# robert80203/HuPR-A-Benchmark-for-Human-Pose-Estimation-Using-Millimeter-Wave-Radar

Hardware: AMD Instinct MI355X
Metric: radar frames/sec (FFT->heatmap fwd+bwd) (higher is better)
Workload: dtype bf16

## Files before the change

hupr-a-benchmark-for-human-pose-estimation-using-millimeter-wave-radar_amd/csrc/conv_halo.h:

```cpp
#pragma once
#include "gemm_common.h"

namespace hupr {

typedef __bf16 bf16x8 __attribute__((ext_vector_type(8)));
typedef unsigned u32x4 __attribute__((ext_vector_type(4)));
typedef float f32x4n __attribute__((ext_vector_type(4)));

typedef __bf16 bf16x4 __attribute__((ext_vector_type(4)));

struct HaloArgs {
    const void* x;
    const __bf16* wp;
    const float* bias;
    const void* res;
    void* y;
    int Bn, D, H, W, Ci, in_ld, Co, out_ld, res_ld;
    int kd;
    int TD, log2TW;
    int nd, nh, nw;
    int n_co_tiles;
    int ablate;
    unsigned long long* trace;
    double* stats;
    float* part;
    int units_per_slice;
    int no_res_prefetch;
};

__device__ __forceinline__ void halo_store_partial(const HaloArgs& p, const f32x16& acc, long m, int chb, int slice) {
    const long M = (long)p.Bn * p.D * p.H * p.W;
    float* dst = p.part + ((long)slice * M + m) * p.Co;
#pragma unroll
    for (int g = 0; g < 4; ++g) {
        const int ch = chb + 8 * g;
        if (ch < p.Co) *reinterpret_cast<f32x4n*>(dst + ch) = (f32x4n){acc[4 * g], acc[4 * g + 1], acc[4 * g + 2], acc[4 * g + 3]};
    }
}

enum HaloRoute {
    kRouteCi32 = 1,
    kRouteCo32 = 2,
    kRoute1x16x16 = 3,
    kRouteStats4x8x8One = 4,
    kRouteStats4x8x8Two = 5,
    kRouteStats2x8x16 = 6,
    kRoute4x8x8 = 7,
    kRoute2x8x16 = 8,
    kRoute128 = 256,
};

int conv_halo256_route(HaloArgs& a, int Bn, bool abf);
void launch_conv_halo256(const HaloArgs& a, int route, hipStream_t s);
bool conv_halo256_supported(const HaloArgs& a, int Bn, bool abf);
bool conv_halo256_stats_ok(const HaloArgs& a, int Bn);
void set_halo_tiles(int mask);
constexpr int kHalo256Grid = 256;

template <bool ABF>
__device__ __forceinline__ void halo_store_voxel(const HaloArgs& p, const f32x16& acc, long m, int chb) {
    if constexpr (ABF) {
        if ((p.Co & 7) == 0 && (p.out_ld & 7) == 0) {
            const int lh = (chb >> 2) & 1, cb = chb - 4 * lh;
            unsigned pk[4][2];
#pragma unroll
            for (int g = 0; g < 4; ++g) {
                f32x4n v = {acc[4 * g], acc[4 * g + 1], acc[4 * g + 2], acc[4 * g + 3]};
                const int ch = chb + 8 * g;
                if (p.bias && ch < p.Co) v += (f32x4n){p.bias[ch], p.bias[ch + 1], p.bias[ch + 2], p.bias[ch + 3]};
                if (p.res && ch < p.Co) {
                    const bf16x4 rv = *reinterpret_cast<const bf16x4*>(static_cast<const __bf16*>(p.res) + m * p.res_ld + ch);
                    v += (f32x4n){(float)rv[0], (float)rv[1], (float)rv[2], (float)rv[3]};
                }
                typedef __bf16 bf16x2 __attribute__((ext_vector_type(2)));
                const bf16x2 lo = {(__bf16)v[0], (__bf16)v[1]}, hi = {(__bf16)v[2], (__bf16)v[3]};
                pk[g][0] = __builtin_bit_cast(unsigned, lo);
                pk[g][1] = __builtin_bit_cast(unsigned, hi);
            }
#pragma unroll
            for (int gp = 0; gp < 4; gp += 2) {
                const auto r0 = __builtin_amdgcn_permlane32_swap(pk[gp][0], pk[gp + 1][0], false, false);
                const auto r1 = __builtin_amdgcn_permlane32_swap(pk[gp][1], pk[gp + 1][1], false, false);
                const int ch = cb + 8 * (gp + lh);
                if (ch < p.Co)
                    *reinterpret_cast<u32x4*>(static_cast<__bf16*>(p.y) + m * p.out_ld + ch) = (u32x4){r0[0], r1[0], r0[1], r1[1]};
            }
            return;
        }
    }
// ... 41 lines not shown
```

hupr-a-benchmark-for-human-pose-estimation-using-millimeter-wave-radar_amd/csrc/conv_halo256m_bf16.hip:

```cpp
#include "conv_halo.h"

namespace hupr {

typedef float f32x4c __attribute__((ext_vector_type(4)));

template <int TD, int TH, int TW, int KD, int NCOT = 0, int NWN = 2, int KC = 64>
__global__ __launch_bounds__(512) void hupr_k_conv_halo256m_bf16(HaloArgs p) {
    constexpr int LDK = KC, BN = 32 * NWN, TS = KC == 64 ? 3 : 9, C8 = KC / 8, L2C8 = KC == 64 ? 3 : 2;
    static_assert(KC == 64 || (KC == 32 && KD == 3 && NWN == 2 && NCOT == 0), "32-channel rows: 3 x 3 x 3 taps, 64 output channels per tile");
    constexpr int HD = TD + KD - 1, HH = TH + 2, HW = TW + 2;
    static_assert(TD * TH * TW == 64 * (8 / NWN) && TH % 8 == 0 && TW % 8 == 0 && (KD == 1 || KD == 3) && (NWN == 2 || NCOT == 0),
                  "256 (512) voxels per tile, 8 x 8 per wave");
    constexpr int NVOX = HD * HH * HW;
    constexpr int T = 9 * KD, NSTAGE = KC == 64 ? 3 * KD : KD, NTAP = KC == 64 ? 6 : 9;
    constexpr bool FULLD = NWN == 1;
    constexpr int NVOXL = FULLD ? TD * HH * HW : NVOX, VOX0 = FULLD ? HH * HW : 0;
    constexpr int NH = (NVOXL * C8 + 511) / 512;
    constexpr int Y0 = NH < NTAP - 1 ? NH : NTAP - 1, Y1 = NH - (NTAP - 1) < 0 ? 0 : (NH - (NTAP - 1) > NTAP ? NTAP : NH - (NTAP - 1)),
                  Y2 = NH - (2 * NTAP - 1) < 0 ? 0 : (NH - (2 * NTAP - 1) > NTAP ? NTAP : NH - (2 * NTAP - 1));
    static_assert(NH <= NTAP * NSTAGE - 1 && NH <= 3 * NTAP - 1, "halo items must all be issued in front of the item's last barrier (and within three stages)");
    __shared__ __attribute__((aligned(16))) __bf16 Hs[(KC == 32 ? 2 : 1) * NVOX * LDK];
    __shared__ __attribute__((aligned(16))) __bf16 Bs[2][TS][BN * LDK];
    constexpr bool STATS = NCOT > 0 && KD == 3;
    constexpr bool SINGLE = STATS && TD == 2;
    f32x4c ssum[STATS ? NCOT : 1][2], ssq[STATS ? NCOT : 1][2];
    if constexpr (!SINGLE) {
#pragma unroll
        for (int ct = 0; ct < (STATS ? NCOT : 1); ++ct)
#pragma unroll
            for (int cg = 0; cg < 2; ++cg) { ssum[ct][cg] = (f32x4c){0.f, 0.f, 0.f, 0.f}; ssq[ct][cg] = (f32x4c){0.f, 0.f, 0.f, 0.f}; }
    }

    const int tid = threadIdx.x, lane = tid & 63, wave = tid >> 6;
    if (wave >= 4) __builtin_amdgcn_s_setprio(1);
    const int wm = NWN == 2 ? wave >> 1 : wave, wn = NWN == 2 ? wave & 1 : 0;
    constexpr int NBX = TW / 8, NBY = TH / 8;
    const int xw0 = 8 * (wm % NBX), yw0 = 8 * ((wm / NBX) % NBY), dzw = wm / (NBX * NBY);
    const int idx = lane & 15, kq = lane >> 4, yy = idx >> 3, wx = idx & 7;
    const int n_tiles = p.Bn * p.nd * p.nh * p.nw * p.n_co_tiles;

    const int wrow_ = NWN == 2 ? 8 * wave + (lane >> 3) : ((8 * wave + (lane >> 3)) & 31);
    const int wsrc_lane = (wrow_ * T * p.Ci + (((lane & 7) ^ (wrow_ >> 1)) & 7) * 8) * 2 +
                          (NWN == 2 ? 0 : (wave >> 2) * (3 * p.Ci * 2));
    constexpr int NDMA = NWN == 2 ? TS : 2, DMA_TAPS = NWN == 2 ? 1 : 2;
    const int wrow32_ = 16 * (wave & 3) + (lane >> 2);
    const int wsrc32_lane = (wrow32_ * T * p.Ci + (((lane & 3) ^ (((wrow32_ >> 3) & 1) << 1)) & 3) * 8) * 2;
    const u32x4 wrs = {(unsigned)(unsigned long)p.wp, (unsigned)((unsigned long)p.wp >> 32) & 0xffffu,
                       (unsigned)((long)p.Co * T * p.Ci * 2), 0x00020000u};
    const unsigned bs_lds = (unsigned)(unsigned long)(__attribute__((address_space(3))) void*)&Bs[0][0][0];
    const unsigned wdst_wave = __builtin_amdgcn_readfirstlane(bs_lds + wave * 1024);
#define HUPR_W_DMA(COT_, CH_, S_, PAR_)                                                                             \
    if constexpr (KC == 32) {                                                                                       \
        _Pragma("unroll") for (int j = 0; j < 5; ++j) {                                                             \
            if (j < 4 || wave < 4) {                                                                                \
                const int t9_ = 2 * j + (wave >> 2);                                  \
                const int wb32_ = (((COT_) * BN * T + (S_) * 9 + (t9_ % 3) * 3 + t9_ / 3) * p.Ci + (CH_) * KC) * 2 + wsrc32_lane; \
                unsigned keep_;                                                                                     \
                asm volatile("s_mov_b32 %0, m0\n\ts_mov_b32 m0, %1\n\ts_nop 0\n\tbuffer_load_dwordx4 %2, %3, 0 offen lds\n\t" \
                             "s_mov_b32 m0, %0"                                                                     \
                             : "=&s"(keep_)                                                                         \
                             : "s"(wdst_wave + (PAR_) * TS * (BN * LDK * 2) + j * 8192), "v"(wb32_), "s"(wrs)       \
                             : "memory");                                                                           \
            }                                                                                                       \
        }                                                                                                           \
    } else {                                                                                                        \
        const int wbase_ = (((COT_) * BN * T + ((S_) / 3) * 9 + ((S_) % 3)) * p.Ci + (CH_) * KC) * 2 + wsrc_lane;   \
        _Pragma("unroll") for (int j = 0; j < NDMA; ++j) {                                                          \
            if (NWN == 2 || j == 0 || wave < 4) {                                                                   \
                unsigned keep_;                                                                                     \
                asm volatile("s_mov_b32 %0, m0\n\ts_mov_b32 m0, %1\n\ts_nop 0\n\tbuffer_load_dwordx4 %2, %3, 0 offen lds\n\t" \
                             "s_mov_b32 m0, %0"                                                                     \
                             : "=&s"(keep_)                                                                         \
                             : "s"(NWN == 2 ? wdst_wave + ((PAR_) * TS + j) * (BN * LDK * 2)                        \
                                            : wdst_wave + (PAR_) * TS * (BN * LDK * 2) + j * 8192),                 \
                               "v"(NWN == 2 ? wbase_ + j * (3 * p.Ci * 2) : wbase_ + j * DMA_TAPS * (3 * p.Ci * 2)), "s"(wrs) \
                             : "memory");                                                                           \
            }                                                                                                       \
        }                                                                                                           \
    }

    u32x4 vb[NH];
    const __amdgpu_buffer_rsrc_t xrs = __builtin_amdgcn_make_buffer_rsrc(
        const_cast<void*>(p.x), 0, (int)((long)p.Bn * p.D * p.H * p.W * p.in_ld * 2), 0x00020000);
#define HUPR_HALO_ISSUE_ITEM(u, COND_, B_, D0_, H0_, W0_, C0_)                                                     \
    {                                                                                                               \
        const int it = tid + (u) * 512;                                                                             \
        const int vox = it >> L2C8, c8 = it & (C8 - 1);                                                             \
        const int hx = vox % HW;                                                                                    \
        const int t_ = vox / HW;                                                                                    \
        const int hy = t_ % HH, hz = t_ / HH;                                                                       \
        const int d = (D0_) + hz - (FULLD ? 0 : KD / 2), h = (H0_) + hy - 1, w = (W0_) + hx - 1;                    \
        const bool ok = (COND_) && it < NVOXL * C8 && (unsigned)d < (unsigned)p.D && (unsigned)h < (unsigned)p.H && \
                        (unsigned)w < (unsigned)p.W;                                                                \
        const int off = (((((B_) * p.D + d) * p.H + h) * p.W + w) * p.in_ld + (C0_) + c8 * 8) * 2;                  \
        const auto ld_ = __builtin_amdgcn_raw_buffer_load_b128(xrs, ok ? off : 0x7ffffff0, 0, 0);                  \
        vb[u] = (u32x4){ld_[0], ld_[1], ld_[2], ld_[3]};                                                            \
    }
#define HUPR_HALO_COMMIT()                                                                                          \
    _Pragma("unroll") for (int u = 0; u < NH; ++u) {                                                                \
        const int it = tid + u * 512;                                                                               \
        if (it < NVOXL * C8) {                                                                                      \
            const int vox = it >> L2C8, c8 = it & (C8 - 1);                                                         \
            const int hx = vox % HW;                                                                                \
            const int key_ = KC == 64 ? (((hx >> 1) & 3) << 1) : ((((vox / HW) % HH) & 1) << 1);                    \
            *reinterpret_cast<u32x4*>(&Hs[(vox + VOX0) * LDK + ((c8 ^ key_) << 3)]) = vb[u];                        \
        }                                                                                                           \
    }

    struct Pos { int cot, twi, thi, tdi, b, ch; };
    const int n_chunks = p.Ci / KC;
    const int per_wg = (n_tiles + gridDim.x - 1) / gridDim.x;
    const int wg_rank = (int)((blockIdx.x & 7) * (gridDim.x >> 3) + (blockIdx.x >> 3));
    const int t_begin = wg_rank * per_wg, t_end = min(n_tiles, t_begin + per_wg);
    if (STATS && p.stats) {
        if (t_begin >= t_end) {
            for (int c = tid; c < 2 * p.Co; c += 512) p.stats[(long)blockIdx.x * 2 * p.Co + c] = 0.0;
        }
    }
    if (t_begin >= t_end) return;
    Pos cur;
    {
        cur.cot = t_begin % p.n_co_tiles;
        int st = t_begin / p.n_co_tiles;
        cur.twi = st % p.nw; st /= p.nw;
        cur.thi = st % p.nh; st /= p.nh;
        cur.tdi = st % p.nd;
        cur.b = st / p.nd;
        cur.ch = 0;
    }
    const int n_items = (t_end - t_begin) * n_chunks;
    const int cot0 = cur.cot;

    int woff[2][2];
#pragma unroll
    for (int cg = 0; cg < 2; ++cg)
#pragma unroll
        for (int kk = 0; kk < 2; ++kk) {
            const int n = 32 * wn + 16 * cg + idx;
            woff[cg][kk] = KC == 64 ? n * LDK + (((4 * kk + kq) ^ ((n >> 1) & 7)) << 3) : n * LDK + ((kq ^ (((n >> 3) & 1) << 1)) << 3);
        }
    const int xlane = ((dzw * HH + yw0 + yy) * HW + xw0 + wx) * LDK;
#define HUPR_HALO_COMMIT1(u, HW_)                                                                                   \
    {                                                                                                               \
        const int it = tid + (u) * 512;                                                                             \
        if (it < NVOXL * C8) {                                                                                      \
            const int vox = it >> L2C8, c8 = it & (C8 - 1);                                                         \
            const int key_ = (((vox / HW) % HH) & 1) << 1;                                                          \
            *reinterpret_cast<u32x4*>(&Hs[(HW_) + (vox + VOX0) * LDK + ((c8 ^ key_) << 3)]) = vb[u];                \
        }                                                                                                           \
    }
#define HUPR_XF(ST_, RHO_, KK_)                                                                                     \
    (KC == 64 ? *reinterpret_cast<const bf16x8*>(&Hs[xlane + ((((ST_) / 3) * HH + (RHO_)) * HW + ((ST_) % 3)) * LDK + \
                    (((4 * (KK_) + kq) ^ ((((xw0 + wx + ((ST_) % 3)) >> 1) & 3) << 1)) << 3)])                      \
              : *reinterpret_cast<const bf16x8*>(&Hs[hrd + xlane + (((ST_) * HH + (RHO_)) * HW + (KK_)) * LDK +     \
                    ((kq ^ (((yy + (RHO_)) & 1) << 1)) << 3)]))
#define HUPR_WF(BUF_, KY_, CG_, KK_)                                                                                \
    (KC == 64 ? *reinterpret_cast<const bf16x8*>(&Bs[BUF_][KY_][woff[CG_][KK_]])                                    \
              : *reinterpret_cast<const bf16x8*>(&Bs[BUF_][3 * (KK_) + (KY_)][woff[CG_][0]]))

    f32x4c c[4][2];
    unsigned accP[4][2][2];
    __bf16* pP = nullptr;
    bool pend = false;
    constexpr bool RESPF = !STATS && TD != 2 && NWN == 2;
    const bool res_pf = RESPF && p.res != nullptr && (p.res_ld & 3) == 0 && !p.no_res_prefetch;
    constexpr bool BIASPF = KC == 32;
    const bool defer = (!p.bias || BIASPF) && (!p.res || res_pf) && (p.Co & 7) == 0 && (p.out_ld & 7) == 0;
    float biasv[BIASPF ? 2 : 1][4];
    bf16x4 resv[4][2];
    constexpr int NB = KC == 64 ? 2 : 3;
    bf16x8 xq[NB][4], x8, wq[NB][2];
#define HUPR_LOAD_TAP(ST_, TAU_, BUF_, WX_)                                                                         \
    {                                                                                                               \
        constexpr int kk_ = (TAU_) / 3, ky_ = (TAU_) % 3;                                                           \
        if ((WX_) & 1) {                                                                                            \
            wq[(TAU_) % NB][0] = HUPR_WF(BUF_, ky_, 0, kk_);                                                        \
            wq[(TAU_) % NB][1] = HUPR_WF(BUF_, ky_, 1, kk_);                                                        \
        }                                                                                                           \
        if ((WX_) & 2) {                                                                                            \
            if (ky_ == 0) { _Pragma("unroll") for (int vg = 0; vg < 4; ++vg) xq[kk_ % NB][vg] = HUPR_XF(ST_, 2 * vg, kk_); } \
            else if (ky_ == 1) { _Pragma("unroll") for (int vg = 0; vg < 4; ++vg) xq[(kk_ + 1) % NB][vg] = HUPR_XF(ST_, 2 * vg + 1, kk_); } \
            else { x8 = HUPR_XF(ST_, 8, kk_); }                                                                     \
        }                                                                                                           \
    }
#define HUPR_VMCNT_LGKM0(N_) __builtin_amdgcn_s_waitcnt(0x0070 | ((N_) & 15) | (((N_) >> 4) << 14))

    if constexpr (FULLD) {
        for (int i = tid; i < 2 * HH * HW * C8; i += 512) {
            const int pl = i / (HH * HW * C8), r = i - pl * (HH * HW * C8);
            *reinterpret_cast<u32x4*>(&Hs[pl * (HD - 1) * HH * HW * LDK + r * 8]) = (u32x4){0u, 0u, 0u, 0u};
// ... 21 lines not shown
        Pos nxt = cur;
        if (++nxt.ch == n_chunks) {
            nxt.ch = 0;
            if (++nxt.cot == p.n_co_tiles) {
                nxt.cot = 0;
                if (++nxt.twi == p.nw) {
                    nxt.twi = 0;
                    if (++nxt.thi == p.nh) {
                        nxt.thi = 0;
                        if (++nxt.tdi == p.nd) { nxt.tdi = 0; ++nxt.b; }
                    }
                }
            }
        }
        const bool has_next = q + 1 < n_items;
        if constexpr (KC == 32) hrd = (q & 1) * (NVOX * LDK);
        [[maybe_unused]] const int hwr = NVOX * LDK - hrd;
        if (first_chunk) {
#pragma unroll
            for (int vg = 0; vg < 4; ++vg)
#pragma unroll
                for (int cg = 0; cg < 2; ++cg) c[vg][cg] = (f32x4c){0.f, 0.f, 0.f, 0.f};
            if constexpr (BIASPF) {
                if (p.bias && defer) {
#pragma unroll
                    for (int cg = 0; cg < 2; ++cg)
#pragma unroll
                        for (int r = 0; r < 4; ++r) biasv[cg][r] = p.bias[n0 + 32 * wn + 16 * cg + 4 * kq + r];
                }
            }
        }
#pragma unroll
        for (int st_ = 0; st_ < NSTAGE; ++st_) {
            const int par = (g + st_) & 1;
#pragma unroll
            for (int tau = 0; tau < NTAP; ++tau) {
                const int kk = tau / 3, ky = tau % 3;
                if (tau == NTAP - 1) {
                    if (st_ == 0) { if (pend) { HUPR_VMCNT_LGKM0(Y0 + 4); } else { HUPR_VMCNT_LGKM0(Y0); } }
                    else if (st_ == 1) { HUPR_VMCNT_LGKM0(Y1); }
                    else if (st_ == 2) { HUPR_VMCNT_LGKM0(Y2); }
                    else { HUPR_VMCNT_LGKM0(0); }
                    __syncthreads();
                    if (st_ + 2 < NSTAGE) { HUPR_W_DMA(cur.cot, cur.ch, st_ + 2, par) }
                    else if (has_next) { HUPR_W_DMA(nxt.cot, nxt.ch, st_ + 2 - NSTAGE, par) }
                    if (KC == 64 && st_ == NSTAGE - 1 && has_next) { HUPR_HALO_COMMIT() }
                }
                if (tau == 0) { HUPR_LOAD_TAP(st_, 1, par, 3) }
                else if (tau == 1) { HUPR_LOAD_TAP(st_, 2, par, 3) }
                else if (tau == 2) { HUPR_LOAD_TAP(st_, 3, par, 3) }
                else if (tau == 3) { HUPR_LOAD_TAP(st_, 4, par, 3) }
                else if (tau == 4) { HUPR_LOAD_TAP(st_, 5, par, 3) }
                else if (NTAP == 9 && tau == 5) { if constexpr (NTAP == 9) { HUPR_LOAD_TAP(st_, 6, par, 3) } }
                else if (NTAP == 9 && tau == 6) { if constexpr (NTAP == 9) { HUPR_LOAD_TAP(st_, 7, par, 3) } }
                else if (NTAP == 9 && tau == 7) { if constexpr (NTAP == 9) { HUPR_LOAD_TAP(st_, 8, par, 3) } }
                else if (st_ + 1 < NSTAGE) { HUPR_LOAD_TAP((st_ + 1) % NSTAGE, 0, par ^ 1, 3) }
                else if (has_next) {
                    if constexpr (KC == 32) { const int hrd = hwr; HUPR_LOAD_TAP(0, 0, par ^ 1, 3) }
                    else { HUPR_LOAD_TAP(0, 0, par ^ 1, 1) }
                }
#pragma unroll
                for (int vg = 0; vg < 4; ++vg) {
                    const bf16x8 xf = ky == 0 ? xq[kk % NB][vg] : (ky == 1 ? xq[(kk + 1) % NB][vg] : (vg < 3 ? xq[kk % NB][vg + 1] : x8));
                    c[vg][0] = __builtin_amdgcn_mfma_f32_16x16x32_bf16(wq[tau % NB][0], xf, c[vg][0], 0, 0, 0);
                    c[vg][1] = __builtin_amdgcn_mfma_f32_16x16x32_bf16(wq[tau % NB][1], xf, c[vg][1], 0, 0, 0);
                }
                if (st_ == 0 && pend && tau < 4) {
// ... 136 lines not shown
#pragma unroll
            for (int cg = 0; cg < 2; ++cg) {
                *reinterpret_cast<f32x4c*>(&St[wave][lane][4 * cg]) = ssum[ct][cg];
                *reinterpret_cast<f32x4c*>(&St[wave][lane][8 + 4 * cg]) = ssq[ct][cg];
            }
            __syncthreads();
            if (tid < 2 * BN) {
                const int k = tid >> 6, ch = tid & 63;
                const int wn_ = ch >> 5, cg = (ch >> 4) & 1, kq_ = (ch >> 2) & 3, r = ch & 3;
                double t = 0.0;
#pragma unroll
                for (int wm_ = 0; wm_ < 4; ++wm_)
#pragma unroll
                    for (int i = 0; i < 16; ++i) t += (double)St[2 * wm_ + wn_][16 * kq_ + i][8 * k + 4 * cg + r];
                p.stats[(long)blockIdx.x * 2 * p.Co + k * p.Co + 64 * ((cot0 + ct) % p.n_co_tiles) + ch] = t;
            }
        }
        if (tid < 2 * BN) {
            const int k = tid >> 6, ch = tid & 63;
            for (int ct = NCOT; ct < p.n_co_tiles; ++ct)
                p.stats[(long)blockIdx.x * 2 * p.Co + k * p.Co + 64 * ((cot0 + ct) % p.n_co_tiles) + ch] = 0.0;
        }
    }
#undef HUPR_W_DMA
#undef HUPR_HALO_ISSUE_ITEM
#undef HUPR_HALO_COMMIT
#undef HUPR_HALO_COMMIT1
#undef HUPR_XF
#undef HUPR_WF
#undef HUPR_LOAD_TAP
#undef HUPR_VMCNT_LGKM0
}

void launch_conv_halo256(const HaloArgs& a, int route, hipStream_t s) {
    const dim3 grid(kHalo256Grid), wg(512);
    switch (route) {
    case kRouteCi32: HUPR_LAUNCH((hupr_k_conv_halo256m_bf16<4, 8, 8, 3, 0, 2, 32>), grid, wg, 0, s, a); break;
    case kRouteCo32: HUPR_LAUNCH((hupr_k_conv_halo256m_bf16<8, 8, 8, 3, 0, 1>), grid, wg, 0, s, a); break;
    case kRoute1x16x16: HUPR_LAUNCH((hupr_k_conv_halo256m_bf16<1, 16, 16, 1>), grid, wg, 0, s, a); break;
    case kRouteStats4x8x8One: HUPR_LAUNCH((hupr_k_conv_halo256m_bf16<4, 8, 8, 3, 1>), grid, wg, 0, s, a); break;
    case kRouteStats4x8x8Two: HUPR_LAUNCH((hupr_k_conv_halo256m_bf16<4, 8, 8, 3, 2>), grid, wg, 0, s, a); break;
    case kRouteStats2x8x16: HUPR_LAUNCH((hupr_k_conv_halo256m_bf16<2, 8, 16, 3, 1>), grid, wg, 0, s, a); break;
    case kRoute4x8x8: HUPR_LAUNCH((hupr_k_conv_halo256m_bf16<4, 8, 8, 3>), grid, wg, 0, s, a); break;
    case kRoute2x8x16: HUPR_LAUNCH((hupr_k_conv_halo256m_bf16<2, 8, 16, 3>), grid, wg, 0, s, a); break;
    }
}

static int g_halo_tiles = 31;
void set_halo_tiles(int mask) { g_halo_tiles = mask & 31; }

static bool offsets_fit(const HaloArgs& a, int Bn) { return (long)Bn * a.D * a.H * a.W * a.in_ld * 2 < 0x7ffffff0L; }

bool conv_halo256_supported(const HaloArgs& a, int Bn, bool abf) {
    if (!abf || !(g_halo_tiles & 1)) return false;
    if (a.kd != 3 || a.D % 4 != 0 || a.H % 8 != 0 || a.W % 8 != 0 || a.Ci % 64 != 0 || a.Co % 64 != 0) return false;
    const long tiles = (long)Bn * (a.D / 4) * (a.H / 8) * (a.W / 8) * (a.Co / 64);
    if (tiles >= (1L << 31) || tiles < 256) return false;
    return offsets_fit(a, Bn);
}

bool conv_halo256_stats_ok(const HaloArgs& a, int Bn) {
    if (a.kd != 3 || a.Ci % 64 != 0 || a.Co % 64 != 0 || !offsets_fit(a, Bn)) return false;
    const int n = a.Co / 64;
    if (a.D % 4 == 0) {
        if (!conv_halo256_supported(a, Bn, true)) return false;
        if (n == 1) return true;
        const long tiles = (long)Bn * (a.D / 4) * (a.H / 8) * (a.W / 8) * n;
        const long per_wg = (tiles + kHalo256Grid - 1) / kHalo256Grid;
        return n <= 2 || per_wg == 1;
    }
    if (!(g_halo_tiles & 2) || a.D % 2 != 0 || a.H % 8 != 0 || a.W % 16 != 0) return false;
    return (long)Bn * (a.D / 2) * (a.H / 8) * (a.W / 16) * n == 256;
}

int conv_halo256_route(HaloArgs& a, int Bn, bool abf) {
    if (!abf || !offsets_fit(a, Bn)) return 0;
    if (a.Ci == 32) {
// ... 48 lines not shown
```

hupr-a-benchmark-for-human-pose-estimation-using-millimeter-wave-radar_amd/csrc/conv_halo_bf16.hip:

```cpp
#include "conv_halo.h"

namespace hupr {



template <int BN, int KC, bool ABF, bool IS3D>
__global__ __launch_bounds__(256, 2) void hupr_k_conv_halo_bf16(HaloArgs p) {
    constexpr bool SWZ = (KC == 64);
    constexpr int LDK = SWZ ? KC : KC + 8;
    constexpr int WN = (BN == 64) ? 2 : 1, WM = 4 / WN;
    constexpr int TM = (128 / WM) / 32;
    constexpr int C8 = KC / 8;
    constexpr int TS = 3;
    constexpr int B_LD = (TS * BN * C8 + 255) / 256;
    constexpr int TD = IS3D ? 2 : 1, TW = IS3D ? 8 : 16, KD = IS3D ? 3 : 1;
    constexpr int HD = TD + KD - 1, HH = 10, HW = TW + 2;
    constexpr int NVOX = HD * HH * HW;
    constexpr int T = KD * 9;
    constexpr int NI = (NVOX * C8 + 255) / 256;

    __shared__ __attribute__((aligned(16))) __bf16 Hs[NVOX * LDK];
    __shared__ __attribute__((aligned(16))) __bf16 Bs[TS][BN * LDK];

    const int tid = threadIdx.x, lane = tid & 63, wave = tid >> 6;
// ... 296 lines not shown
            src = ((long)co * d.ci + ci) * d.taps + (d.taps - 1 - tapf);
        }
        const float v = d.w[src];
        void* dst = pb.layout ? d.wp1 : d.wp0;
        if (d.kind == 1) static_cast<__bf16*>(dst)[l] = (__bf16)v;
        else static_cast<float*>(dst)[l] = v;
    }
}

}

using namespace hupr;

extern "C" int hupr_pack_conv_weights_table(const void* descs_dev, const void* blocks_dev, int n_blocks, hupr_stream_t stream) {
    HUPR_REQUIRE(descs_dev && blocks_dev && n_blocks > 0, "hupr_pack_conv_weights_table: bad argument");
    static_assert(sizeof(PackDesc) == 48 && sizeof(PackBlock) == 16, "PackDesc / PackBlock layouts are part of the ABI");
    HUPR_LAUNCH(hupr_k_pack_table, dim3((unsigned)n_blocks), dim3(256), 0, as_stream(stream),
                       reinterpret_cast<const PackDesc*>(descs_dev), reinterpret_cast<const PackBlock*>(blocks_dev));
    HUPR_LAUNCH_OK("hupr_k_pack_table");
    return HUPR_OK;
}

extern "C" int hupr_pack_conv_weights_bf16(const float* w, void* wp_bf16, int Co, int Ci, int taps, int mode,
                                           hupr_stream_t stream) {
    HUPR_REQUIRE(w && wp_bf16 && Co > 0 && Ci > 0 && taps > 0 && (mode == 0 || mode == 1),
                 "hupr_pack_conv_weights_bf16: bad argument");
    const long n = (long)Co * Ci * taps;
    HUPR_LAUNCH(hupr_k_pack_weights_bf16, dim3((n + 255) / 256), dim3(256), 0, as_stream(stream), w,
                       reinterpret_cast<__bf16*>(wp_bf16), Co, Ci, taps, mode);
    HUPR_LAUNCH_OK("hupr_k_pack_weights_bf16");
    return HUPR_OK;
}

static int g_halo_ablate = 0;
static int g_halo_variant = 0;
static unsigned long long* g_halo_trace = nullptr;
extern "C" void hupr_debug_halo_trace(void* buf) { g_halo_trace = reinterpret_cast<unsigned long long*>(buf); }
extern "C" void hupr_debug_halo_ablate(int bits) { g_halo_ablate = bits; }
extern "C" void hupr_debug_halo_variant(int v) { g_halo_variant = v; }
extern "C" void hupr_debug_halo_tiles(int mask) { set_halo_tiles(mask); }
static int g_halo_split_k = 1;
extern "C" void hupr_debug_halo_split_k(int on) { g_halo_split_k = on; }

extern "C" int hupr_conv3x3_halo_supported(int D, int H, int W, int Ci, int kd, int kh, int kw, int pd, int ph, int pw) {
    if (kh != 3 || kw != 3 || ph != 1 || pw != 1) return 0;
    if (!((kd == 3 && pd == 1) || (kd == 1 && pd == 0))) return 0;
    if (Ci % 32 != 0 || H % 8 != 0) return 0;
    if (kd == 3) return (D % 2 == 0 && W % 8 == 0) ? 1 : 0;
    return (D == 1 && W % 16 == 0) ? 1 : 0;
}

static int halo_k_slices(int Bn, int D, int H, int W, int Ci, int Co, int kd, int* units_per_slice) {
    *units_per_slice = 0;
    if (!g_halo_split_k || !hupr_conv3x3_halo_supported(D, H, W, Ci, kd, 3, 3, kd / 2, 1, 1) || Co % 32 != 0) return 1;
    const int td = kd == 3 ? 2 : 1, tw = kd == 3 ? 8 : 16;
    const long tiles = (long)Bn * (D / td) * (H / 8) * (W / tw);
    if (tiles * ((Co + 63) / 64) > 256) return 1;
    const long blocks = tiles * (Co / 32);
    const int units = (Ci / (Ci % 64 == 0 ? 64 : 32)) * (kd == 3 ? 3 : 1);
    if (blocks >= 384 || units < 2) return 1;
    int s = (int)min((long)units, (768 + blocks - 1) / blocks);
    const int per = (units + s - 1) / s;
    s = (units + per - 1) / per;
    *units_per_slice = per;
    return s;
}

static int g_halo_no_res_prefetch = 0;
extern "C" void hupr_debug_halo_res_prefetch(int on) { g_halo_no_res_prefetch = on ? 0 : 1; }

static int halo_plan(HaloArgs& a, bool abf, size_t ws_bytes, bool partial_only, int* n_slices, const char* who) {
    const int Bn = a.Bn, D = a.D, H = a.H, W = a.W, Ci = a.Ci, Co = a.Co, kd = a.kd;
    *n_slices = 1;
// ... 13 lines not shown
        if (route) return route;
    }
    if (kd == 3) { a.TD = 2; a.log2TW = 3; } else { a.TD = 1; a.log2TW = 4; }
    a.nd = D / a.TD; a.nh = H / 8; a.nw = W >> a.log2TW;
    const long blocks64 = (long)Bn * a.nd * a.nh * a.nw * ((Co + 63) / 64);
    const bool n32 = (Co <= 32) || (blocks64 <= 256 && Co % 32 == 0);
    const int bn = n32 ? 32 : 64;
    a.n_co_tiles = (Co + bn - 1) / bn;
    const long blocks = (long)Bn * a.nd * a.nh * a.nw * a.n_co_tiles;
    HUPR_REQUIRE(blocks < (1L << 31), "%s: grid too large", who);
    if (ws_bytes && abf && n32) {
        int per = 0;
        const int want = halo_k_slices(Bn, D, H, W, Ci, Co, kd, &per);
        const size_t need = (size_t)want * Bn * D * H * W * Co * sizeof(float);
        if (want > 1 && ws_bytes >= need) {
            *n_slices = want;
            a.units_per_slice = per;
        }
    }
    HUPR_REQUIRE(!partial_only || *n_slices > 1,
                 "%s: this geometry is not K-sliced (hupr_conv3x3_halo_splitk_ws_bytes() == 0) or the workspace is too small", who);
    return kRoute128 + 16 * *n_slices + 8 * (bn == 64) + 4 * (Ci % 64 == 0) + 2 * (kd == 3) + (abf ? 1 : 0);
}

static int conv3x3_halo(const void* x, const void* wp_bf16, const float* bias, const void* res, void* y, int Bn, int D,
                        int H, int W, int Ci, int in_ld, int Co, int out_ld, int res_ld, int kd, bool abf,
                        hupr_stream_t stream, const char* who, double* stats = nullptr, void* ws = nullptr, size_t ws_bytes = 0,
                        bool partial_only = false) {
    HUPR_REQUIRE(x && wp_bf16 && y, "%s: null pointer", who);
    HaloArgs a;
    a.x = x; a.wp = reinterpret_cast<const __bf16*>(wp_bf16); a.bias = bias; a.res = res; a.y = y;
    a.Bn = Bn; a.D = D; a.H = H; a.W = W; a.Ci = Ci; a.in_ld = in_ld; a.Co = Co; a.out_ld = out_ld; a.res_ld = res_ld;
    a.kd = kd;
    a.ablate = g_halo_ablate;
    a.trace = g_halo_trace;
    a.stats = stats;
    a.part = nullptr;
    a.units_per_slice = 0;
    a.no_res_prefetch = g_halo_no_res_prefetch;
    int n_slices = 1;
    const int route = halo_plan(a, abf, (ws && ((uintptr_t)ws & 15) == 0) ? ws_bytes : 0, partial_only, &n_slices, who);
    if (route < 0) return route;
    hipStream_t s = as_stream(stream);
    if (route < kRoute128) {
        launch_conv_halo256(a, route, s);
        HUPR_LAUNCH_OK(stats ? "hupr_k_conv_halo256m_bf16<stats>" : "hupr_k_conv_halo256m_bf16");
        return HUPR_OK;
    }
    if (n_slices > 1) a.part = static_cast<float*>(ws);
    const long blocks = (long)Bn * a.nd * a.nh * a.nw * a.n_co_tiles;
#define HUPR_HALO_LAUNCH(BN_, KC_)                                                                                       \
    do {                                                                                                                 \
        const dim3 grid_((unsigned)blocks, (unsigned)n_slices);                                                          \
        if (kd == 3) {                                                                                                   \
            if (abf) HUPR_LAUNCH((hupr_k_conv_halo_bf16<BN_, KC_, true, true>), grid_, dim3(256), 0, s, a);       \
            else HUPR_LAUNCH((hupr_k_conv_halo_bf16<BN_, KC_, false, true>), grid_, dim3(256), 0, s, a);          \
        } else {                                                                                                         \
            if (abf) HUPR_LAUNCH((hupr_k_conv_halo_bf16<BN_, KC_, true, false>), grid_, dim3(256), 0, s, a);      \
            else HUPR_LAUNCH((hupr_k_conv_halo_bf16<BN_, KC_, false, false>), grid_, dim3(256), 0, s, a);         \
        }                                                                                                                \
    } while (0)
    const bool n32 = !(route & 8);
    if (route & 4) {
        if (n32) HUPR_HALO_LAUNCH(32, 64); else HUPR_HALO_LAUNCH(64, 64);
    } else {
        if (n32) HUPR_HALO_LAUNCH(32, 32); else HUPR_HALO_LAUNCH(64, 32);
    }
// ... 26 lines not shown
                        "hupr_conv3x3_halo_bf16");
}

extern "C" int hupr_conv3x3_halo_bf16act(const void* x, const void* wp_bf16, const float* bias, const void* res, void* y,
                                         int Bn, int D, int H, int W, int Ci, int in_ld, int Co, int out_ld, int res_ld,
                                         int kd, hupr_stream_t stream) {
    return conv3x3_halo(x, wp_bf16, bias, res, y, Bn, D, H, W, Ci, in_ld, Co, out_ld, res_ld, kd, true, stream,
                        "hupr_conv3x3_halo_bf16act");
}

extern "C" size_t hupr_conv3x3_halo_splitk_ws_bytes(int Bn, int D, int H, int W, int Ci, int Co, int kd) {
    int per = 0;
    if (Bn <= 0 || D <= 0 || H <= 0 || W <= 0 || Ci <= 0 || Co <= 0) return 0;
    const int s = halo_k_slices(Bn, D, H, W, Ci, Co, kd, &per);
    return s > 1 ? (size_t)s * Bn * D * H * W * Co * sizeof(float) : 0;
}
extern "C" int hupr_conv3x3_halo_bf16act_ws(const void* x, const void* wp_bf16, const float* bias, const void* res, void* y,
                                            int Bn, int D, int H, int W, int Ci, int in_ld, int Co, int out_ld, int res_ld,
                                            int kd, void* ws, size_t ws_bytes, hupr_stream_t stream) {
    return conv3x3_halo(x, wp_bf16, bias, res, y, Bn, D, H, W, Ci, in_ld, Co, out_ld, res_ld, kd, true, stream,
                        "hupr_conv3x3_halo_bf16act_ws", nullptr, ws, ws_bytes);
}

extern "C" int hupr_conv3x3_halo_bf16act_partial(const void* x, const void* wp_bf16, int Bn, int D, int H, int W, int Ci, int in_ld,
                                                 int Co, int kd, void* part, size_t part_bytes, hupr_stream_t stream) {
    HUPR_REQUIRE(part, "hupr_conv3x3_halo_bf16act_partial: null pointer");
    return conv3x3_halo(x, wp_bf16, nullptr, nullptr, part , Bn, D, H, W, Ci, in_ld, Co,
                        Co, 0, kd, true, stream, "hupr_conv3x3_halo_bf16act_partial", nullptr, part, part_bytes, true);
}

extern "C" int hupr_conv3x3_halo_stats_supported(int Bn, int D, int H, int W, int Ci, int Co, int kd) {
    HaloArgs a{};
    a.kd = kd; a.D = D; a.H = H; a.W = W; a.Ci = Ci; a.Co = Co; a.in_ld = Ci;
    a.ablate = g_halo_ablate; a.trace = g_halo_trace;
    return (Bn > 0 && conv_halo256_stats_ok(a, Bn)) ? 1 : 0;
}
extern "C" int hupr_conv3x3_halo_stats_rows(void) { return kHalo256Grid; }
extern "C" int hupr_conv3x3_halo_bf16act_stats(const void* x, const void* wp_bf16, void* y, int Bn, int D, int H, int W, int Ci,
                                               int in_ld, int Co, int out_ld, int kd, void* stats, hupr_stream_t stream) {
    HUPR_REQUIRE(stats, "hupr_conv3x3_halo_bf16act_stats: null pointer");
    return conv3x3_halo(x, wp_bf16, nullptr, nullptr, y, Bn, D, H, W, Ci, in_ld, Co, out_ld, 0, kd, true, stream,
                        "hupr_conv3x3_halo_bf16act_stats", static_cast<double*>(stats));
}
```

hupr-a-benchmark-for-human-pose-estimation-using-millimeter-wave-radar_amd/runtime.py:

```python
import ctypes
import os

import torch

_HERE = os.path.dirname(os.path.abspath(__file__))
LIB_PATH = os.path.join(_HERE, "lib", "libhupr_hip.so")

c_void_p, c_int, c_size_t, c_float, c_char_p = (ctypes.c_void_p, ctypes.c_int, ctypes.c_size_t,
                                                ctypes.c_float, ctypes.c_char_p)
c_long = ctypes.c_long

class AttnItem(ctypes.Structure):
    _fields_ = [("K", ctypes.c_void_p), ("Q", ctypes.c_void_p), ("V", ctypes.c_void_p), ("Vres", ctypes.c_void_p),
                ("out", ctypes.c_void_p), ("lse", ctypes.c_void_p), ("out16", ctypes.c_void_p)]


class SumItem(ctypes.Structure):
    _fields_ = [("partial", ctypes.c_void_p), ("n", ctypes.c_int), ("out", ctypes.c_void_p)]


class AttnBwdItem(ctypes.Structure):
    _fields_ = [(n, ctypes.c_void_p) for n in ("K", "Q", "V", "dO", "V32", "out", "lse", "dK", "dQ", "dV", "Dq")] + \
               [("residual", ctypes.c_int), ("accumulate", ctypes.c_int)]

# ... 11 lines not shown
    "hupr_stream_state_bytes": (c_size_t, []),
    "hupr_stream_reset": (c_int, [c_void_p, c_void_p]),
    "hupr_stream_advance": (c_int, [c_void_p, c_int, c_int, c_void_p]),
    "hupr_mnet_stream_f32": (c_int, [c_void_p] * 3 + [c_int, c_int] + [c_void_p] * 6 + [c_int] * 3 + [c_void_p]),
    "hupr_mnet_stream_bf16act": (c_int, [c_void_p] * 3 + [c_int, c_int] + [c_void_p] * 6 + [c_int] * 3 + [c_void_p]),
    "hupr_stream_keypoints_f32": (c_int, [c_void_p] * 3 + [c_long, c_int, c_float, c_void_p]),
    "hupr_pose_filter_state_bytes": (c_size_t, [c_long]),
    "hupr_pose_decode_f32": (c_int, [c_void_p, c_long, c_int, c_int, c_float, c_int, c_void_p] + [c_float] * 5 + [c_void_p] * 6),
    "hupr_fft_chain_opts": (c_int, [c_void_p, c_int, c_void_p, c_int, c_int, c_void_p, c_size_t, c_void_p]),
    "hupr_loader_normalize_c64": (c_int, [c_void_p, c_int, c_void_p, c_void_p]),
    "hupr_dca1000_deinterleave": (c_int, [c_void_p, c_void_p, c_int, c_void_p]),
    "hupr_gemm_f32": (c_int, [c_int, c_int, c_void_p, c_void_p, c_void_p, c_int, c_int, c_int, c_long, c_long,
                              c_long, c_int, c_long, c_long, c_long, c_void_p, c_long, c_long, c_int, c_void_p]),
    "hupr_conv_fwd_f32": (c_int, [c_void_p] * 5 + [c_int] * 19 + [c_void_p]),
    "hupr_conv_wgrad_ws_bytes": (c_size_t, [c_int] * 9),
    "hupr_conv_wgrad_f32": (c_int, [c_void_p] * 3 + [c_int] * 17 + [c_void_p, c_size_t, c_void_p]),
    "hupr_gemm_bf16": (c_int, [c_int, c_int, c_void_p, c_void_p, c_void_p, c_int, c_int, c_int, c_long, c_long,
                               c_long, c_int, c_long, c_long, c_long, c_void_p, c_long, c_long, c_int, c_void_p]),
    "hupr_conv_fwd_bf16": (c_int, [c_void_p] * 5 + [c_int] * 19 + [c_void_p]),
    "hupr_conv_wgrad_bf16": (c_int, [c_void_p] * 3 + [c_int] * 17 + [c_void_p, c_size_t, c_void_p]),
    "hupr_conv_fwd_bf16_mixed": (c_int, [c_void_p, c_int, c_void_p, c_void_p, c_void_p, c_int] + [c_int] * 17 + [c_void_p]),
    "hupr_conv_wgrad_bf16_mixed": (c_int, [c_void_p, c_int, c_void_p, c_void_p] + [c_int] * 17
                                   + [c_void_p, c_size_t, c_void_p]),
    "hupr_tmerge_dgrad_bf16": (c_int, [c_void_p, c_void_p, c_void_p, c_int] + [c_int] * 5 + [c_void_p]),
    "hupr_pack_conv_weights_bf16": (c_int, [c_void_p, c_void_p, c_int, c_int, c_int, c_int, c_void_p]),
    "hupr_conv3x3_halo_stats_supported": (c_int, [c_int] * 7),
    "hupr_conv3x3_halo_stats_rows": (c_int, []),
    "hupr_conv3x3_halo_bf16act_stats": (c_int, [c_void_p, c_void_p, c_void_p] + [c_int] * 9 + [c_void_p, c_void_p]),
    "hupr_bn_train_finalize_f32": (c_int, [c_void_p, c_int, c_long, c_int] + [c_void_p] * 4 + [c_float, c_float] + [c_void_p] * 5),
    "hupr_bn_train_finalize2_f32": (c_int, ([c_void_p, c_int] + [c_void_p] * 4 + [c_float, c_float] + [c_void_p] * 4) * 2
                                    + [c_long, c_int, c_void_p]),
    "hupr_pack_conv_weights_table": (c_int, [c_void_p, c_void_p, c_int, c_void_p]),
    "hupr_debug_attn_trace": (None, [c_void_p]),
    "hupr_debug_halo_ablate": (None, [c_int]),
    "hupr_debug_halo_variant": (None, [c_int]),
    "hupr_debug_halo_tiles": (None, [c_int]),
    "hupr_debug_halo_trace": (None, [c_void_p]),
    "hupr_debug_wgrad_ci32": (None, [c_int]),
    "hupr_debug_wgrad_m16": (None, [c_int]),
    "hupr_debug_splitk_slices": (None, [c_int]),
    "hupr_debug_halo_res_prefetch": (None, [c_int]),
    "hupr_debug_halo_route": (c_int, [c_int] * 12),
    "hupr_debug_wgrad_route": (c_int, [c_int] * 11 + [c_size_t, ctypes.POINTER(c_int)]),
    "hupr_conv3x3_halo_supported": (c_int, [c_int] * 10),
    "hupr_conv3x3_halo_bf16": (c_int, [c_void_p] * 5 + [c_int] * 10 + [c_void_p]),
    "hupr_conv3x3_wgrad_halo_ws_bytes": (c_size_t, [c_int, c_int, c_int]),
    "hupr_conv3x3_wgrad_halo_bf16": (c_int, [c_void_p] * 3 + [c_int] * 9 + [c_void_p, c_size_t, c_void_p]),
    "hupr_pack_conv_weights_f32": (c_int, [c_void_p, c_void_p, c_int, c_int, c_int, c_int, c_void_p]),
    "hupr_bn_ws_bytes": (c_size_t, [c_int]),
    "hupr_bn_train_stats_f32": (c_int, [c_void_p, c_long, c_int, c_void_p, c_void_p, c_void_p, c_void_p, c_float,
                                        c_float, c_void_p, c_void_p, c_void_p, c_void_p, c_void_p, c_size_t, c_void_p]),
    "hupr_bn_eval_params_f32": (c_int, [c_void_p] * 4 + [c_float, c_int, c_void_p, c_void_p, c_void_p]),
    "hupr_scale_shift_act_f32": (c_int, [c_void_p] * 7 + [c_long, c_int, c_int, c_void_p]),
    "hupr_bn_eval_act_f32": (c_int, [c_void_p] * 5 + [c_float] + [c_void_p] * 5 + [c_float, c_void_p, c_long, c_int, c_int, c_void_p]),
    "hupr_bn_eval_act_bf16act": (c_int, [c_void_p] * 5 + [c_float] + [c_void_p] * 5 + [c_float, c_void_p, c_long, c_int, c_int, c_void_p]),
    "hupr_bn_bwd_f32": (c_int, [c_void_p] * 9 + [c_long, c_int, c_int, c_void_p, c_size_t, c_void_p]),
    "hupr_bn_bwd2_f32": (c_int, [c_void_p] * 16 + [c_long, c_int, c_int, c_void_p, c_size_t, c_void_p]),
    "hupr_bn_bwd_remask_f32": (c_int, [c_void_p] * 10 + [c_long, c_int, c_int, c_void_p, c_size_t, c_void_p]),
    "hupr_bn_bwd_remask_bf16act": (c_int, [c_void_p] * 10 + [c_long, c_int, c_int, c_void_p, c_size_t, c_void_p]),
    "hupr_bn_bwd2_remask_f32": (c_int, [c_void_p] * 19 + [c_long, c_int, c_int, c_void_p, c_size_t, c_void_p]),
    "hupr_bn_bwd2_remask_bf16act": (c_int, [c_void_p] * 19 + [c_long, c_int, c_int, c_void_p, c_size_t, c_void_p]),
    "hupr_bn_bwd2_bf16act": (c_int, [c_void_p] * 16 + [c_long, c_int, c_int, c_void_p, c_size_t, c_void_p]),
    "hupr_colsum_f32": (c_int, [c_void_p, c_long, c_int, c_void_p, c_void_p, c_size_t, c_void_p]),
    "hupr_prelu_fwd_f32": (c_int, [c_void_p, c_void_p, c_void_p, c_long, c_void_p]),
    "hupr_prelu_ws_bytes": (c_size_t, []),
    "hupr_prelu_bwd_f32": (c_int, [c_void_p] * 5 + [c_long, c_void_p, c_size_t, c_void_p]),
    "hupr_mnet_fwd_f32": (c_int, [c_void_p] * 5 + [c_long, c_int, c_void_p]),
    "hupr_mnet_bwd_ws_bytes": (c_size_t, []),
    "hupr_mnet_bwd_f32": (c_int, [c_void_p] * 7 + [c_long, c_int, c_void_p, c_size_t, c_void_p]),
# ... 165 lines not shown
```

include/hupr_debug.h:

```cpp
#ifndef HUPR_DEBUG_H
#define HUPR_DEBUG_H
#include <stddef.h>
#ifdef __cplusplus
extern "C" {
#endif

void hupr_debug_attn_trace(void* dev_buf);
void hupr_debug_halo_variant(int v);
void hupr_debug_halo_ablate(int bits);
void hupr_debug_halo_res_prefetch(int on);
void hupr_debug_splitk_slices(int s);
void hupr_debug_wgrad_m16(int on);
void hupr_debug_wgrad_ci32(int on);
void hupr_debug_halo_trace(void* device_u64_4096);
void hupr_debug_attn_split(int mode);
void hupr_debug_halo_split_k(int on);
void hupr_debug_halo_tiles(int mask);

int hupr_debug_halo_route(int Bn, int D, int H, int W, int Ci, int in_ld, int Co, int out_ld, int kd, int abf, int stats, int sliced_ws);
int hupr_debug_wgrad_route(int Bn, int D, int H, int W, int Ci, int in_ld, int Co, int dy_ld, int kd, int abf, int dual, size_t ws_bytes,
                           int* groups_out);
#ifdef __cplusplus
}
#endif
#endif
```

Baseline: 1711.

## Add two-plane halo conv variant for depth-2 volumes, skipping padded depth halo

Adds a two-plane specialization of the 2x8x16 halo conv kernel, used when the input depth is exactly 2 and there is a single depth tile. The halo buffer holds only the two real planes instead of four padded ones. The weight DMA instead loads six tap images, one per depth offset each output plane needs, so each wave reads its own weights and the depth halo loads (which would be out of range anyway) are skipped. It also drops the unused ablate debug hook. The cost is a larger weight double buffer in shared memory and a different stage and parity schedule, which may affect occupancy or correctness.

```diff
diff --git a/hupr-a-benchmark-for-human-pose-estimation-using-millimeter-wave-radar_amd/csrc/conv_halo.h b/hupr-a-benchmark-for-human-pose-estimation-using-millimeter-wave-radar_amd/csrc/conv_halo.h
--- a/hupr-a-benchmark-for-human-pose-estimation-using-millimeter-wave-radar_amd/csrc/conv_halo.h
+++ b/hupr-a-benchmark-for-human-pose-estimation-using-millimeter-wave-radar_amd/csrc/conv_halo.h
@@ -55,6 +55,7 @@
 bool conv_halo256_supported(const HaloArgs& a, int Bn, bool abf);
 bool conv_halo256_stats_ok(const HaloArgs& a, int Bn);
 void set_halo_tiles(int mask);
+void set_halo_two_plane(int on);
 constexpr int kHalo256Grid = 256;
 
 template <bool ABF>
diff --git a/hupr-a-benchmark-for-human-pose-estimation-using-millimeter-wave-radar_amd/csrc/conv_halo256m_bf16.hip b/hupr-a-benchmark-for-human-pose-estimation-using-millimeter-wave-radar_amd/csrc/conv_halo256m_bf16.hip
--- a/hupr-a-benchmark-for-human-pose-estimation-using-millimeter-wave-radar_amd/csrc/conv_halo256m_bf16.hip
+++ b/hupr-a-benchmark-for-human-pose-estimation-using-millimeter-wave-radar_amd/csrc/conv_halo256m_bf16.hip
@@ -4,15 +4,17 @@
 
 typedef float f32x4c __attribute__((ext_vector_type(4)));
 
-template <int TD, int TH, int TW, int KD, int NCOT = 0, int NWN = 2, int KC = 64>
+template <int TD, int TH, int TW, int KD, int NCOT = 0, int NWN = 2, int KC = 64, bool TP = false>
 __global__ __launch_bounds__(512) void hupr_k_conv_halo256m_bf16(HaloArgs p) {
     constexpr int LDK = KC, BN = 32 * NWN, TS = KC == 64 ? 3 : 9, C8 = KC / 8, L2C8 = KC == 64 ? 3 : 2;
     static_assert(KC == 64 || (KC == 32 && KD == 3 && NWN == 2 && NCOT == 0), "32-channel rows: 3 x 3 x 3 taps, 64 output channels per tile");
-    constexpr int HD = TD + KD - 1, HH = TH + 2, HW = TW + 2;
+    static_assert(!TP || (TD == 2 && KD == 3 && NWN == 2 && KC == 64), "two-plane form: the 2 x 8 x 16 tile at D == 2 (launcher: nd == 1)");
+    constexpr int NIMG = TP ? 2 * TS : TS;
+    constexpr int HD = TP ? TD : TD + KD - 1, HH = TH + 2, HW = TW + 2;
     static_assert(TD * TH * TW == 64 * (8 / NWN) && TH % 8 == 0 && TW % 8 == 0 && (KD == 1 || KD == 3) && (NWN == 2 || NCOT == 0),
                   "256 (512) voxels per tile, 8 x 8 per wave");
     constexpr int NVOX = HD * HH * HW;
-    constexpr int T = 9 * KD, NSTAGE = KC == 64 ? 3 * KD : KD, NTAP = KC == 64 ? 6 : 9;
+    constexpr int T = 9 * KD, NSTAGE = TP ? 6 : (KC == 64 ? 3 * KD : KD), NTAP = KC == 64 ? 6 : 9;
     constexpr bool FULLD = NWN == 1;
     constexpr int NVOXL = FULLD ? TD * HH * HW : NVOX, VOX0 = FULLD ? HH * HW : 0;
     constexpr int NH = (NVOXL * C8 + 511) / 512;
@@ -20,7 +22,7 @@
                   Y2 = NH - (2 * NTAP - 1) < 0 ? 0 : (NH - (2 * NTAP - 1) > NTAP ? NTAP : NH - (2 * NTAP - 1));
     static_assert(NH <= NTAP * NSTAGE - 1 && NH <= 3 * NTAP - 1, "halo items must all be issued in front of the item's last barrier (and within three stages)");
     __shared__ __attribute__((aligned(16))) __bf16 Hs[(KC == 32 ? 2 : 1) * NVOX * LDK];
-    __shared__ __attribute__((aligned(16))) __bf16 Bs[2][TS][BN * LDK];
+    __shared__ __attribute__((aligned(16))) __bf16 Bs[2][NIMG][BN * LDK];
     constexpr bool STATS = NCOT > 0 && KD == 3;
     constexpr bool SINGLE = STATS && TD == 2;
     f32x4c ssum[STATS ? NCOT : 1][2], ssq[STATS ? NCOT : 1][2];
@@ -42,7 +44,7 @@
     const int wrow_ = NWN == 2 ? 8 * wave + (lane >> 3) : ((8 * wave + (lane >> 3)) & 31);
     const int wsrc_lane = (wrow_ * T * p.Ci + (((lane & 7) ^ (wrow_ >> 1)) & 7) * 8) * 2 +
                           (NWN == 2 ? 0 : (wave >> 2) * (3 * p.Ci * 2));
-    constexpr int NDMA = NWN == 2 ? TS : 2, DMA_TAPS = NWN == 2 ? 1 : 2;
+    constexpr int NDMA = NWN == 2 ? NIMG : 2, DMA_TAPS = NWN == 2 ? 1 : 2;
     const int wrow32_ = 16 * (wave & 3) + (lane >> 2);
     const int wsrc32_lane = (wrow32_ * T * p.Ci + (((lane & 3) ^ (((wrow32_ >> 3) & 1) << 1)) & 3) * 8) * 2;
     const u32x4 wrs = {(unsigned)(unsigned long)p.wp, (unsigned)((unsigned long)p.wp >> 32) & 0xffffu,
@@ -67,13 +69,17 @@
         const int wbase_ = (((COT_) * BN * T + ((S_) / 3) * 9 + ((S_) % 3)) * p.Ci + (CH_) * KC) * 2 + wsrc_lane;   \
         _Pragma("unroll") for (int j = 0; j < NDMA; ++j) {                                                          \
             if (NWN == 2 || j == 0 || wave < 4) {                                                                   \
+                 \
+                               \
+                const int tap_ = (j < 3 ? 9 : 0) + 3 * (j % 3);                                                     \
                 unsigned keep_;                                                                                     \
                 asm volatile("s_mov_b32 %0, m0\n\ts_mov_b32 m0, %1\n\ts_nop 0\n\tbuffer_load_dwordx4 %2, %3, 0 offen lds\n\t" \
                              "s_mov_b32 m0, %0"                                                                     \
                              : "=&s"(keep_)                                                                         \
-                             : "s"(NWN == 2 ? wdst_wave + ((PAR_) * TS + j) * (BN * LDK * 2)                        \
+                             : "s"(NWN == 2 ? wdst_wave + ((PAR_) * NIMG + j) * (BN * LDK * 2)                      \
                                             : wdst_wave + (PAR_) * TS * (BN * LDK * 2) + j * 8192),                 \
-                               "v"(NWN == 2 ? wbase_ + j * (3 * p.Ci * 2) : wbase_ + j * DMA_TAPS * (3 * p.Ci * 2)), "s"(wrs) \
+                               "v"(TP ? wbase_ + tap_ * (p.Ci * 2)                                                  \
+                                      : (NWN == 2 ? wbase_ + j * (3 * p.Ci * 2) : wbase_ + j * DMA_TAPS * (3 * p.Ci * 2))), "s"(wrs) \
                              : "memory");                                                                           \
             }                                                                                                       \
         }                                                                                                           \
@@ -89,7 +95,7 @@
         const int hx = vox % HW;                                                                                    \
         const int t_ = vox / HW;                                                                                    \
         const int hy = t_ % HH, hz = t_ / HH;                                                                       \
-        const int d = (D0_) + hz - (FULLD ? 0 : KD / 2), h = (H0_) + hy - 1, w = (W0_) + hx - 1;                    \
+        const int d = (D0_) + hz - (FULLD || TP ? 0 : KD / 2), h = (H0_) + hy - 1, w = (W0_) + hx - 1;                    \
         const bool ok = (COND_) && it < NVOXL * C8 && (unsigned)d < (unsigned)p.D && (unsigned)h < (unsigned)p.H && \
                         (unsigned)w < (unsigned)p.W;                                                                \
         const int off = (((((B_) * p.D + d) * p.H + h) * p.W + w) * p.in_ld + (C0_) + c8 * 8) * 2;                  \
@@ -138,8 +144,9 @@
         for (int kk = 0; kk < 2; ++kk) {
             const int n = 32 * wn + 16 * cg + idx;
             woff[cg][kk] = KC == 64 ? n * LDK + (((4 * kk + kq) ^ ((n >> 1) & 7)) << 3) : n * LDK + ((kq ^ (((n >> 3) & 1) << 1)) << 3);
-        }
-    const int xlane = ((dzw * HH + yw0 + yy) * HW + xw0 + wx) * LDK;
+            if constexpr (TP) woff[cg][kk] += dzw * (TS * BN * LDK);
+        }
+    const int xlane = (((TP ? 0 : dzw) * HH + yw0 + yy) * HW + xw0 + wx) * LDK;
 #define HUPR_HALO_COMMIT1(u, HW_)                                                                                   \
     {                                                                                                               \
         const int it = tid + (u) * 512;                                                                             \
@@ -155,7 +162,8 @@
               : *reinterpret_cast<const bf16x8*>(&Hs[hrd + xlane + (((ST_) * HH + (RHO_)) * HW + (KK_)) * LDK +     \
                     ((kq ^ (((yy + (RHO_)) & 1) << 1)) << 3)]))
 #define HUPR_WF(BUF_, KY_, CG_, KK_)                                                                                \
-    (KC == 64 ? *reinterpret_cast<const bf16x8*>(&Bs[BUF_][KY_][woff[CG_][KK_]])                                    \
+    (TP ? *reinterpret_cast<const bf16x8*>(&Bs[0][0][0] + ((BUF_) * NIMG + (KY_)) * (BN * LDK) + woff[CG_][KK_])    \
+     : KC == 64 ? *reinterpret_cast<const bf16x8*>(&Bs[BUF_][KY_][woff[CG_][KK_]])                                  \
               : *reinterpret_cast<const bf16x8*>(&Bs[BUF_][3 * (KK_) + (KY_)][woff[CG_][0]]))
 
     f32x4c c[4][2];
@@ -243,7 +251,7 @@
         }
 #pragma unroll
         for (int st_ = 0; st_ < NSTAGE; ++st_) {
-            const int par = (g + st_) & 1;
+            const int par = TP ? (st_ & 1) : ((g + st_) & 1);
 #pragma unroll
             for (int tau = 0; tau < NTAP; ++tau) {
                 const int kk = tau / 3, ky = tau % 3;
@@ -446,17 +454,27 @@
 #undef HUPR_VMCNT_LGKM0
 }
 
+static int g_halo_two_plane = 1;
+void set_halo_two_plane(int on) { g_halo_two_plane = on; }
+
 void launch_conv_halo256(const HaloArgs& a, int route, hipStream_t s) {
     const dim3 grid(kHalo256Grid), wg(512);
+    const bool tp = g_halo_two_plane && a.TD == 2 && a.D == 2 && a.nd == 1;
     switch (route) {
     case kRouteCi32: HUPR_LAUNCH((hupr_k_conv_halo256m_bf16<4, 8, 8, 3, 0, 2, 32>), grid, wg, 0, s, a); break;
     case kRouteCo32: HUPR_LAUNCH((hupr_k_conv_halo256m_bf16<8, 8, 8, 3, 0, 1>), grid, wg, 0, s, a); break;
     case kRoute1x16x16: HUPR_LAUNCH((hupr_k_conv_halo256m_bf16<1, 16, 16, 1>), grid, wg, 0, s, a); break;
     case kRouteStats4x8x8One: HUPR_LAUNCH((hupr_k_conv_halo256m_bf16<4, 8, 8, 3, 1>), grid, wg, 0, s, a); break;
     case kRouteStats4x8x8Two: HUPR_LAUNCH((hupr_k_conv_halo256m_bf16<4, 8, 8, 3, 2>), grid, wg, 0, s, a); break;
-    case kRouteStats2x8x16: HUPR_LAUNCH((hupr_k_conv_halo256m_bf16<2, 8, 16, 3, 1>), grid, wg, 0, s, a); break;
+    case kRouteStats2x8x16:
+        if (tp) HUPR_LAUNCH((hupr_k_conv_halo256m_bf16<2, 8, 16, 3, 1, 2, 64, true>), grid, wg, 0, s, a);
+        else HUPR_LAUNCH((hupr_k_conv_halo256m_bf16<2, 8, 16, 3, 1>), grid, wg, 0, s, a);
+        break;
     case kRoute4x8x8: HUPR_LAUNCH((hupr_k_conv_halo256m_bf16<4, 8, 8, 3>), grid, wg, 0, s, a); break;
-    case kRoute2x8x16: HUPR_LAUNCH((hupr_k_conv_halo256m_bf16<2, 8, 16, 3>), grid, wg, 0, s, a); break;
+    case kRoute2x8x16:
+        if (tp) HUPR_LAUNCH((hupr_k_conv_halo256m_bf16<2, 8, 16, 3, 0, 2, 64, true>), grid, wg, 0, s, a);
+        else HUPR_LAUNCH((hupr_k_conv_halo256m_bf16<2, 8, 16, 3>), grid, wg, 0, s, a);
+        break;
     }
 }
 
diff --git a/hupr-a-benchmark-for-human-pose-estimation-using-millimeter-wave-radar_amd/csrc/conv_halo_bf16.hip b/hupr-a-benchmark-for-human-pose-estimation-using-millimeter-wave-radar_amd/csrc/conv_halo_bf16.hip
--- a/hupr-a-benchmark-for-human-pose-estimation-using-millimeter-wave-radar_amd/csrc/conv_halo_bf16.hip
+++ b/hupr-a-benchmark-for-human-pose-estimation-using-millimeter-wave-radar_amd/csrc/conv_halo_bf16.hip
@@ -352,13 +352,12 @@
     return HUPR_OK;
 }
 
-static int g_halo_ablate = 0;
 static int g_halo_variant = 0;
 static unsigned long long* g_halo_trace = nullptr;
 extern "C" void hupr_debug_halo_trace(void* buf) { g_halo_trace = reinterpret_cast<unsigned long long*>(buf); }
-extern "C" void hupr_debug_halo_ablate(int bits) { g_halo_ablate = bits; }
 extern "C" void hupr_debug_halo_variant(int v) { g_halo_variant = v; }
 extern "C" void hupr_debug_halo_tiles(int mask) { set_halo_tiles(mask); }
+extern "C" void hupr_debug_halo_two_plane(int on) { set_halo_two_plane(on); }
 static int g_halo_split_k = 1;
 extern "C" void hupr_debug_halo_split_k(int on) { g_halo_split_k = on; }
 
@@ -438,7 +437,7 @@
     a.x = x; a.wp = reinterpret_cast<const __bf16*>(wp_bf16); a.bias = bias; a.res = res; a.y = y;
     a.Bn = Bn; a.D = D; a.H = H; a.W = W; a.Ci = Ci; a.in_ld = in_ld; a.Co = Co; a.out_ld = out_ld; a.res_ld = res_ld;
     a.kd = kd;
-    a.ablate = g_halo_ablate;
+    a.ablate = 0;
     a.trace = g_halo_trace;
     a.stats = stats;
     a.part = nullptr;
@@ -531,7 +530,7 @@
 extern "C" int hupr_conv3x3_halo_stats_supported(int Bn, int D, int H, int W, int Ci, int Co, int kd) {
     HaloArgs a{};
     a.kd = kd; a.D = D; a.H = H; a.W = W; a.Ci = Ci; a.Co = Co; a.in_ld = Ci;
-    a.ablate = g_halo_ablate; a.trace = g_halo_trace;
+    a.trace = g_halo_trace;
     return (Bn > 0 && conv_halo256_stats_ok(a, Bn)) ? 1 : 0;
 }
 extern "C" int hupr_conv3x3_halo_stats_rows(void) { return kHalo256Grid; }
diff --git a/hupr-a-benchmark-for-human-pose-estimation-using-millimeter-wave-radar_amd/runtime.py b/hupr-a-benchmark-for-human-pose-estimation-using-millimeter-wave-radar_amd/runtime.py
--- a/hupr-a-benchmark-for-human-pose-estimation-using-millimeter-wave-radar_amd/runtime.py
+++ b/hupr-a-benchmark-for-human-pose-estimation-using-millimeter-wave-radar_amd/runtime.py
@@ -67,9 +67,9 @@
                                     + [c_long, c_int, c_void_p]),
     "hupr_pack_conv_weights_table": (c_int, [c_void_p, c_void_p, c_int, c_void_p]),
     "hupr_debug_attn_trace": (None, [c_void_p]),
-    "hupr_debug_halo_ablate": (None, [c_int]),
     "hupr_debug_halo_variant": (None, [c_int]),
     "hupr_debug_halo_tiles": (None, [c_int]),
+    "hupr_debug_halo_two_plane": (None, [c_int]),
     "hupr_debug_halo_trace": (None, [c_void_p]),
     "hupr_debug_wgrad_ci32": (None, [c_int]),
     "hupr_debug_wgrad_m16": (None, [c_int]),
diff --git a/include/hupr_debug.h b/include/hupr_debug.h
--- a/include/hupr_debug.h
+++ b/include/hupr_debug.h
@@ -7,7 +7,6 @@
 
 void hupr_debug_attn_trace(void* dev_buf);
 void hupr_debug_halo_variant(int v);
-void hupr_debug_halo_ablate(int bits);
 void hupr_debug_halo_res_prefetch(int on);
 void hupr_debug_splitk_slices(int s);
 void hupr_debug_wgrad_m16(int on);
@@ -16,6 +15,7 @@
 void hupr_debug_attn_split(int mode);
 void hupr_debug_halo_split_k(int on);
 void hupr_debug_halo_tiles(int mask);
+void hupr_debug_halo_two_plane(int on);
 
 int hupr_debug_halo_route(int Bn, int D, int H, int W, int Ci, int in_ld, int Co, int out_ld, int kd, int abf, int stats, int sliced_ws);
 int hupr_debug_wgrad_route(int Bn, int D, int H, int W, int Ci, int in_ld, int Co, int dy_ld, int kd, int abf, int dual, size_t ws_bytes,
```

Measured after the change: 1729, median of 6. +1.0%, better.
